# vandenheuvel/relp

Hardware: AMD Instinct MI355X
Metric: simplex pivots/sec + wall-clock to optimal, Netlib 25fv47 @1 GPU (higher is better)
Workload: dtype f64; 1 GPU; Netlib 25FV47 821x1876, steepest-edge pricing, explicit-inverse carry, exact certificate inside the timed step, no presolve (+520 virtual artificials); carry=explicit, refactors=0, parallelism=1 LP per GPU x1, certified=True, objective_bits=1791

## Files before the change

relp_amd/csrc/kernels.hip:

```cpp
#include <hip/hip_runtime.h>
#include <hip/hip_ext.h>

#include <cmath>
#include <cstdlib>
#include <string>
#include <utility>

#include "kernels.hpp"
#include "pivot_step.hpp"
#include "price_step.hpp"
#include "solver.hpp"
#include "wave_ops.hpp"

namespace relp {


__global__ void budget_kernel(Ctl* ctl, long long add) {
    if (ctl->status == ST_BUDGET) ctl->status = ST_RUNNING;
    ctl->budget = ctl->iters + add;
}

typedef double f64x2_t __attribute__((ext_vector_type(2)));
template <int RULE, bool USE_LDS, int LPC, bool UNIT = false>
__global__ void __launch_bounds__(256) price_kernel(DeviceLP lp, int skip_weights, double tol_dual, int col_first,
// ... 1796 lines not shown
            ctl->rho_buf ^= 1;
        }
        s_toggle = toggle;
        s_amount = amount;
    }
    __syncthreads();
    const int toggle = s_toggle;
    if (toggle >= 0) {
        const double amount = s_amount;
        for (int e = lp.col_start[toggle] + threadIdx.x; e < lp.col_start[toggle + 1]; e += blockDim.x)
            lp.rhs[lp.row_index[e]] -= amount * lp.value[e];
    }
}

constexpr int K2F_NW = K2F_THREADS / WAVE;
constexpr int K2F_INLINE_BLOCKS = 128;

struct K2fShared {
    double akey[K2F_NW];
    unsigned long long arank[K2F_NW];
    double red[K2F_NW + 2];
    double red2[K2F_NW + 2];
    double cbarv[K2F_MAX_BLOCKS];
    int crows[K2F_INLINE_BLOCKS * ELL_W];
    double cvals[K2F_INLINE_BLOCKS * ELL_W];
    int clen[K2F_INLINE_BLOCKS];
    int rows[K2_COL_CHUNK];
    double vals[K2_COL_CHUNK];
    double bcast[4];
    int ibcast[2];
};
static_assert(K2F_INLINE_BLOCKS * ELL_W <= 2 * K2F_THREADS, "the inline entries are two loads per thread");
struct K2fCandidateLoads {
    int j, len;
    double key, cbar;
    int row[2];
    double val[2];
};
__device__ __forceinline__ void k2f_candidates_issue(const DeviceLP& lp, int n_price_blocks, K2fCandidateLoads& c) {
    const int tid = threadIdx.x;
    const int bc = tid < n_price_blocks ? tid : 0;
    c.j = lp.cand_j[bc];
    c.key = lp.cand_key[bc];
    c.cbar = lp.cand_cbar[bc];
    c.len = lp.cand_len[bc];
#pragma unroll
    for (int t = 0; t < 2; ++t) {
        const int e = tid + t * K2F_THREADS;
        const int ec = e < n_price_blocks * ELL_W ? e : 0;
        c.row[t] = lp.cand_rows[ec];
        c.val[t] = lp.cand_vals[ec];
    }
}
template <int RULE>
__device__ __forceinline__ void k2f_candidates_fold(const DeviceLP& lp, int n_price_blocks, K2fShared& sm, const K2fCandidateLoads& c,
                                                    double& ckey, unsigned long long& crank) {
    const int tid = threadIdx.x;
    if (tid < n_price_blocks) {
        sm.cbarv[tid] = c.cbar;
        offer_entering<RULE>(c.key, c.j, tid, ckey, crank);
    }
    if (n_price_blocks <= K2F_INLINE_BLOCKS) {
#pragma unroll
        for (int t = 0; t < 2; ++t) {
            const int e = tid + t * K2F_THREADS;
            if (e < n_price_blocks * ELL_W) {
                sm.crows[e] = c.row[t];
                sm.cvals[e] = c.val[t];
            }
        }
        if (tid < n_price_blocks) sm.clen[tid] = c.len;
    }
    for (int b = tid + K2F_THREADS; b < n_price_blocks; b += K2F_THREADS) {
        const int j = lp.cand_j[b];
        const double k = lp.cand_key[b];
        const double cb = lp.cand_cbar[b];
        RELP_LOADS_ISSUED();
        sm.cbarv[b] = cb;
        offer_entering<RULE>(k, j, b, ckey, crank);
    }
}
template <int RULE>
__device__ __forceinline__ int k2f_entering(double ckey, unsigned long long crank, K2fShared& sm, double& cbar_q, int& winner_block) {
    const int q = entering_winner<RULE>(ckey, crank, sm.akey, sm.arank, winner_block);
    cbar_q = q >= 0 ? sm.cbarv[winner_block] : 0.0;
    return q;
}
template <int R>
__device__ __forceinline__ void k2f_ftran_inline(const DeviceLP& lp, const double* T, const K2fShared& sm, int q, int winner_block,
                                                 double (&al)[R], int& ca, int& cb_) {
    const int tid = threadIdx.x, m = lp.m, ld = lp.ld;
    const int len = sm.clen[winner_block];
    if (len >= 0) {
        constexpr int G = R <= 4 ? R : 4;
#pragma unroll
        for (int rg = 0; rg < R; rg += G) {
            double t[G][ELL_W];
#pragma unroll
            for (int g = 0; g < G; ++g) {
                const int i = tid + (rg + g) * K2F_THREADS;
                const double* col = T + (i < m ? i : 0);
#pragma unroll
                for (int e = 0; e < ELL_W; ++e) t[g][e] = col[(size_t)sm.crows[winner_block * ELL_W + e] * ld];
            }
            RELP_LOADS_ISSUED();
#pragma unroll
            for (int g = 0; g < G; ++g) {
                double a0 = 0.0;
#pragma unroll
                for (int e = 0; e < ELL_W; ++e) a0 += t[g][e] * sm.cvals[winner_block * ELL_W + e];
                if (tid + (rg + g) * K2F_THREADS < m) al[rg + g] = a0;
            }
        }
    }
    if (len > ELL_W || len < 0) {
        ca = lp.col_start[q] + (len < 0 ? 0 : ELL_W);
        cb_ = lp.col_start[q + 1];
    }
}
template <int R>
__device__ __forceinline__ void k2f_ftran_csc(const DeviceLP& lp, const double* T, K2fShared& sm, int ca, int cb_, double (&al)[R]) {
    const int tid = threadIdx.x, m = lp.m, ld = lp.ld;
    for (int c0 = ca; c0 < cb_; c0 += K2_COL_CHUNK) {
        const int cnt = min(K2_COL_CHUNK, cb_ - c0);
        __syncthreads();
        for (int e = tid; e < cnt; e += K2F_THREADS) {
            sm.rows[e] = lp.row_index[c0 + e];
            sm.vals[e] = lp.value[c0 + e];
        }
        __syncthreads();
        if constexpr (R <= 8) {
            double acc[R][4];
            int row[R];
#pragma unroll
            for (int r = 0; r < R; ++r) {
                const int i = tid + r * K2F_THREADS;
                row[r] = i < m ? i : 0;
                acc[r][0] = acc[r][1] = acc[r][2] = acc[r][3] = 0.0;
            }
            int e = 0;
            for (; e + 4 <= cnt; e += 4) {
                const size_t o0 = (size_t)sm.rows[e] * ld, o1 = (size_t)sm.rows[e + 1] * ld, o2 = (size_t)sm.rows[e + 2] * ld, o3 = (size_t)sm.rows[e + 3] * ld;
                const double v0 = sm.vals[e], v1 = sm.vals[e + 1], v2 = sm.vals[e + 2], v3 = sm.vals[e + 3];
                double x[R][4];
#pragma unroll
                for (int r = 0; r < R; ++r) {
                    x[r][0] = T[o0 + row[r]];
                    x[r][1] = T[o1 + row[r]];
                    x[r][2] = T[o2 + row[r]];
                    x[r][3] = T[o3 + row[r]];
                }
#pragma unroll
                for (int r = 0; r < R; ++r) {
                    acc[r][0] += x[r][0] * v0;
                    acc[r][1] += x[r][1] * v1;
                    acc[r][2] += x[r][2] * v2;
                    acc[r][3] += x[r][3] * v3;
                }
            }
            for (; e < cnt; ++e) {
                const size_t o = (size_t)sm.rows[e] * ld;
                const double v = sm.vals[e];
                double x[R];
#pragma unroll
                for (int r = 0; r < R; ++r) x[r] = T[o + row[r]];
#pragma unroll
                for (int r = 0; r < R; ++r) acc[r][0] += x[r] * v;
            }
#pragma unroll
            for (int r = 0; r < R; ++r)
                if (tid + r * K2F_THREADS < m) al[r] += (acc[r][0] + acc[r][1]) + (acc[r][2] + acc[r][3]);
        } else {
#pragma unroll
            for (int r = 0; r < R; ++r) {
                const int i = tid + r * K2F_THREADS;
                if (i >= m) continue;
                const double* col = T + i;
                double a0 = 0.0, a1 = 0.0, a2 = 0.0, a3 = 0.0;
                int e = 0;
                for (; e + 4 <= cnt; e += 4) {
                    a0 += col[(size_t)sm.rows[e] * ld] * sm.vals[e];
                    a1 += col[(size_t)sm.rows[e + 1] * ld] * sm.vals[e + 1];
                    a2 += col[(size_t)sm.rows[e + 2] * ld] * sm.vals[e + 2];
                    a3 += col[(size_t)sm.rows[e + 3] * ld] * sm.vals[e + 3];
                }
                for (; e < cnt; ++e) a0 += col[(size_t)sm.rows[e] * ld] * sm.vals[e];
                al[r] += (a0 + a1) + (a2 + a3);
            }
        }
    }
}
template <int R>
__device__ __forceinline__ void k2f_pass1(const DeviceLP& lp, bool bounded, const double (&al)[R], const double (&xb)[R], const int (&bas)[R],
                                          double tol_pivot, double slack, int skip_artificial_rows, bool (&eligible)[R], double (&room)[R],
                                          double& sumsq, double& theta) {
    const int tid = threadIdx.x, m = lp.m;
#pragma unroll
    for (int r = 0; r < R; ++r) {
        const int i = tid + r * K2F_THREADS;
        const double a = al[r];
        sumsq += a * a;
        const bool allowed = i < m && !(skip_artificial_rows && bas[r] < lp.n_art);
        const RowRoom row = row_room(a, xb[r], [&] { return lp.xub[i]; }, allowed, bounded, tol_pivot);
        eligible[r] = row.eligible;
        room[r] = row.room;
        if (row.eligible) theta = fmin(theta, harris_pass1(row.room, slack, a));
    }
}
__device__ __forceinline__ void k2f_reduce(K2fShared& sm, double sumsq, double theta, double& gamma_q, double& theta_max) {
    const int lane = threadIdx.x & (WAVE - 1), wave = threadIdx.x / WAVE;
    sumsq = wave_sum(sumsq);
    theta = wave_min(theta);
    if (lane == LAST) {
        sm.red[wave] = sumsq;
        sm.red2[wave] = theta;
    }
    __syncthreads();
    if (wave == 0) {
        double t1 = lane < K2F_NW ? sm.red[lane] : 0.0;
        double t2 = lane < K2F_NW ? sm.red2[lane] : INFINITY;
        t1 = wave_sum(t1);
        t2 = wave_min(t2);
        if (lane == LAST) {
            sm.red[K2F_NW] = t1;
            sm.red2[K2F_NW] = t2;
        }
    }
    __syncthreads();
    gamma_q = 1.0 + sm.red[K2F_NW];
    theta_max = sm.red2[K2F_NW];
}
template <int R>
__device__ __forceinline__ int k2f_pass2(bool textbook, const double (&al)[R], const bool (&eligible)[R], const double (&room)[R],
                                         const int (&bas)[R], double theta_max, K2fShared& sm) {
    double hkey = 0.0;
    unsigned long long hrank = RANK_NONE;
#pragma unroll
    for (int r = 0; r < R; ++r) {
        const double mag = fabs(al[r]);
        if (eligible[r] && harris_accepts(room[r], mag, theta_max))
            keep_better(harris_key(textbook, mag), leaving_rank(bas[r], threadIdx.x + r * K2F_THREADS), hkey, hrank);
    }
    block_argbest(hkey, hrank, sm.akey, sm.arank);
    return leaving_row(hrank);
}
template <int R>
__device__ __forceinline__ void k2f_broadcast_row(int p, const double (&al)[R], const double (&xb)[R], const double (&room)[R],
                                                  const int (&bas)[R], K2fShared& sm) {
#pragma unroll
    for (int r = 0; r < R; ++r) {
        if ((int)threadIdx.x + r * K2F_THREADS == p) {
            sm.bcast[1] = al[r];
            sm.bcast[2] = xb[r];
            sm.bcast[3] = room[r];
            sm.ibcast[0] = bas[r];
        }
    }
    __syncthreads();
}

template <int RULE, int R>
__global__ void __launch_bounds__(K2F_THREADS) ftran_ratio_fast_kernel(DeviceLP lp, int n_price_blocks, double tol_pivot,
                                                                     double harris_delta, int skip_artificial_rows,
                                                                     int mode, int n_alpha_slices) {
    __shared__ K2fShared sm;
    Ctl* ctl = lp.ctl;
    STAMP_INIT;
    const int tid = threadIdx.x;
    const int m = lp.m;
    kernel_args_ready(ctl, lp.xB, lp.basis, lp.alpha_in, lp.cand_j, lp.cand_key, lp.cand_cbar, lp.cand_len, lp.cand_rows, lp.cand_vals, m, n_price_blocks,
                      n_alpha_slices);
    double xb[R];
    int bas[R];
    double ain[R];
    const bool preselected = n_alpha_slices > 0;
    const double* ain_from = preselected ? lp.alpha_in : lp.xB;
#pragma unroll
    for (int r = 0; r < R; ++r) {
        const int i = tid + r * K2F_THREADS;
        const int ic = i < m ? i : 0;
        xb[r] = lp.xB[ic];
        bas[r] = lp.basis[ic];
        ain[r] = ain_from[ic];
    }
    double ckey = 0.0;
    unsigned long long crank = RANK_NONE;
    K2fCandidateLoads cand;
    k2f_candidates_issue(lp, n_price_blocks, cand);
    RELP_LOADS_PINNED();
    const int status = ctl->status;
    const long long iters = ctl->iters;
    const long long budget = ctl->budget;
    const int forced_q = ctl->forced_q;
    const int forced_p = ctl->forced_p;
    const double minus_obj = ctl->minus_obj;
    const int q_loaded = ctl->q;
    const double cbar_loaded = ctl->cbar_q;
    RELP_LOADS_ISSUED();
    const int q_pre = preselected ? q_loaded : -1;
    const double cbar_pre = preselected ? cbar_loaded : 0.0;
#pragma unroll
    for (int r = 0; r < R; ++r) {
        if (tid + r * K2F_THREADS >= m) {
            xb[r] = 0.0;
            bas[r] = 0x7fffffff;
        }
        if (!preselected || tid + r * K2F_THREADS >= m) ain[r] = 0.0;
    }
    if (!preselected) k2f_candidates_fold<RULE>(lp, n_price_blocks, sm, cand, ckey, crank);
    const bool inline_column = forced_q < 0 && !preselected && n_price_blocks <= K2F_INLINE_BLOCKS;
    if (status != ST_RUNNING) return;
    STAMP(0);
    if (mode == 0 && iters >= budget) {
        if (tid == 0) ctl_budget(*ctl);
        return;
    }
    int q;
    double cbar_q;
    int winner_block = 0;
    if (preselected && forced_q < 0) {
        q = q_pre;
        cbar_q = cbar_pre;
    } else if (forced_q < 0) {
        q = k2f_entering<RULE>(ckey, crank, sm, cbar_q, winner_block);
    } else {
        q = forced_q;
// ... 102 lines not shown
        }
        __syncthreads();
        if (wave_k2 == 0) {
            int carry = 0;
#pragma unroll
            for (int base = 0; base < R * NW; base += WAVE) {
                const int c = base + lane_k2 < R * NW ? s_nz_count[base + lane_k2] : 0;
                int incl = c;
#pragma unroll
                for (int d = 1; d < WAVE; d <<= 1) {
                    const int up = __shfl_up(incl, d);
                    if (lane_k2 >= d) incl += up;
                }
                if (base + lane_k2 < R * NW) s_nz_count[base + lane_k2] = carry + incl - c;
                carry += __shfl(incl, WAVE - 1);
            }
            if (lane_k2 == 0) s_nz_count[R * NW] = carry;
        }
        __syncthreads();
#pragma unroll
        for (int r = 0; r < R; ++r) {
            const int i = tid + r * K2F_THREADS;
            if (i < m && (al[r] != 0.0 || i == p)) {
                const int slot = s_nz_count[r * NW + wave_k2] + __popcll(masks[r] & ((1ull << lane_k2) - 1ull));
                lp.nz_index[slot] = i;
                lp.nz_alpha[slot] = al[r];
            }
        }
        total = s_nz_count[R * NW];
    }
#pragma unroll
    for (int r = 0; r < R; ++r) {
        const int i = tid + r * K2F_THREADS;
        if (i < m) {
            lp.alpha[i] = al[r];
            lp.xB[i] = (i == p) ? xp : xb[r] - al[r] * xp;
        }
    }
    STAMP(5);
    const int leaving_flipped = bounded ? lp.flipped[leaving] : 0;
    if (step.leaves_at_upper) {
        const double sgn_l = leaving_flipped ? -1.0 : 1.0;
        for (int e = lp.col_start[leaving] + tid; e < lp.col_start[leaving + 1]; e += K2F_THREADS)
            lp.rhs[lp.row_index[e]] -= step.ub_leaving * sgn_l * lp.value[e];
    }
    if (bounded) __syncthreads();
    if (tid == 0) {
        lp.basis[p] = q;
        push_touched(lp, *ctl, p);
        if (lp.eta_cap > 0) {
            int is_new = 0;
            if (eta_slot_p < 0) {
                const int k = ctl->eta_count;
                lp.eta_slot[p] = k;
                lp.eta_rows[k] = p;
                ctl->eta_count = k + 1;
                is_new = 1;
            }
            ctl->eta_new = is_new;
            ctl->eta_version = ctl->eta_version + 1;
        }
        ctl_basis_change(lp, *ctl, bounded, q, p, leaving, leaving_flipped, step, ub_q, cbar_q, alpha_pq, gamma_q, total, minus_obj, iters);
        ctl->rho_buf ^= 1;
    }
    STAMP(6);
}

constexpr int KF_THREADS = K2F_THREADS;
constexpr int KF_NW = KF_THREADS / WAVE;
template <int RULE, int KF_R>
__global__ void __launch_bounds__(KF_THREADS) pivot_fused_kernel(DeviceLP lp, DeviceLP::State in, DeviceLP::State out, int n_price_blocks,
                                                                 double tol_pivot, double harris_delta, int skip_artificial_rows) {
    constexpr int R = KF_R;
    constexpr int KF_U = KF_R * KF_THREADS / WAVE;
    constexpr int KF_M = KF_R * KF_THREADS;
    __shared__ K2fShared sm;
    __shared__ double s_alpha[KF_M];
    const Ctl* ctl = in.ctl;
    const int tid = threadIdx.x;
    const int lane = tid & (WAVE - 1), wave = tid / WAVE;
#ifdef RELP_STAMPS
    unsigned long long t_prev__ = clock64();
    if (tid == 0 && blockIdx.x == 0) lp.dbg[63] += 1;
#define FSTAMP(k) do { if (tid == 0 && blockIdx.x == 0) { unsigned long long t__ = clock64(); lp.dbg[(k)] += t__ - t_prev__; t_prev__ = t__; } } while (0)
#else
#define FSTAMP(k) do {} while (0)
#endif
    const int m = lp.m, ld = lp.ld;
    const bool writer = blockIdx.x == 0;
    kernel_args_ready(ctl, in.xB, in.basis, lp.cand_j, lp.cand_key, lp.cand_cbar, lp.cand_len, lp.cand_rows, lp.cand_vals, m, n_price_blocks);
    double xb[R];
    int bas[R];
#pragma unroll
    for (int r = 0; r < R; ++r) {
        const int i = tid + r * KF_THREADS;
        const int ic = i < m ? i : 0;
        xb[r] = in.xB[ic];
        bas[r] = in.basis[ic];
    }
    double ckey = 0.0;
    unsigned long long crank = RANK_NONE;
    K2fCandidateLoads cand;
    k2f_candidates_issue(lp, n_price_blocks, cand);
    RELP_LOADS_PINNED();
    const int status = ctl->status;
    const long long iters = ctl->iters;
    const long long budget = ctl->budget;
    const double minus_obj = ctl->minus_obj;
    const int t_buf = ctl->t_buf;
    RELP_LOADS_ISSUED();
#pragma unroll
    for (int r = 0; r < R; ++r) {
        if (tid + r * KF_THREADS >= m) {
            xb[r] = 0.0;
            bas[r] = 0x7fffffff;
        }
    }
    k2f_candidates_fold<RULE>(lp, n_price_blocks, sm, cand, ckey, crank);
    const bool inline_column = n_price_blocks <= K2F_INLINE_BLOCKS;
    auto hand_on = [&](auto verdict) {
        if (!writer) return;
#pragma unroll
        for (int r = 0; r < R; ++r) {
            const int i = tid + r * KF_THREADS;
            if (i < m) {
                out.xB[i] = xb[r];
                out.basis[i] = bas[r];
            }
        }
        if (tid == 0) {
            Ctl c;
            ctl_copy(c, *ctl);
            verdict(c);
            c.forced_q = -1;
            c.forced_p = -1;
            ctl_copy(*out.ctl, c);
        }
    };
    if (status != ST_RUNNING) {
        hand_on([](Ctl&) {});
        return;
    }
    FSTAMP(0);
    if (iters >= budget) {
        hand_on([](Ctl& c) { ctl_budget(c); });
        return;
    }
    const int j_own = blockIdx.x * KF_NW + wave;
    const bool own = j_own < m;
    const double* t_old = (t_buf ? lp.Binv2 : lp.Binv);
    double* t_new = (t_buf ? lp.Binv : lp.Binv2);
    const double* c_old = t_old + (size_t)(own ? j_own : 0) * ld;
    double o[KF_U];
#pragma unroll
    for (int u = 0; u < KF_U; ++u) {
        const int i = lane + u * WAVE;
        o[u] = c_old[i < m ? i : 0];
    }
    double pi_old = lp.minus_pi[own ? j_own : 0];
    RELP_LOADS_PINNED();
    double cbar_q;
    int winner_block = 0;
    const int q = k2f_entering<RULE>(ckey, crank, sm, cbar_q, winner_block);
    if (q < 0) {
        hand_on([](Ctl& c) { ctl_no_entering(c, 0); });
        return;
    }
    FSTAMP(1);
    double al[R];
#pragma unroll
    for (int r = 0; r < R; ++r) al[r] = 0.0;
    int ca = 0, cb_ = 0;
    if (inline_column) {
        k2f_ftran_inline<R>(lp, t_old, sm, q, winner_block, al, ca, cb_);
    } else {
        ca = lp.col_start[q];
        cb_ = lp.col_start[q + 1];
    }
#pragma unroll
    for (int u = 0; u < KF_U; ++u) {
        if (!own || lane + u * WAVE >= m) o[u] = 0.0;
    }
    if (!own || lane != LAST) pi_old = 0.0;
    k2f_ftran_csc<R>(lp, t_old, sm, ca, cb_, al);
    FSTAMP(2);
    const HarrisRule harris = harris_rule(harris_delta);
    double sumsq = 0.0, theta = INFINITY;
    bool eligible[R];
    double room[R];
    k2f_pass1<R>(lp, false, al, xb, bas, tol_pivot, harris.slack, skip_artificial_rows, eligible, room, sumsq, theta);
#pragma unroll
    for (int r = 0; r < R; ++r) s_alpha[tid + r * KF_THREADS] = al[r];
    double gamma_q, theta_max;
    k2f_reduce(sm, sumsq, theta, gamma_q, theta_max);
    FSTAMP(3);
    const int p = k2f_pass2<R>(harris.textbook, al, eligible, room, bas, theta_max, sm);
    if (p < 0) {
        hand_on([q](Ctl& c) { ctl_unbounded(c, q, 0); });
        return;
    }
    FSTAMP(4);
    k2f_broadcast_row<R>(p, al, xb, room, bas, sm);
    const double alpha_pq = sm.bcast[1];
    const int leaving = sm.ibcast[0];
    const Step step = step_decision(false, false, p, alpha_pq, sm.bcast[2], sm.bcast[3], INFINITY);
    const double xp = step.xp;
    if (writer) {
#pragma unroll
        for (int r = 0; r < R; ++r) {
            const int i = tid + r * KF_THREADS;
            if (i < m) {
                lp.alpha[i] = al[r];
                out.xB[i] = (i == p) ? xp : xb[r] - al[r] * xp;
                out.basis[i] = (i == p) ? q : bas[r];
            }
        }
        if (tid == 0) {
            Ctl c;
            ctl_copy(c, *ctl);
            ctl_basis_change(lp, c, false, q, p, leaving, 0, step, INFINITY, cbar_q, alpha_pq, gamma_q, 0, minus_obj, iters);
            c.t_buf = t_buf ^ 1;
            ctl_copy(*out.ctl, c);
        }
    }
    FSTAMP(5);
    if (!own) return;
    const int u_p = p >> 6, lane_p = p & (WAVE - 1);
    double o_p = 0.0;
#pragma unroll
    for (int u = 0; u < KF_U; ++u) o_p = (u == u_p) ? o[u] : o_p;
    const double r_j = __shfl(o_p, lane_p) / alpha_pq;
    double* c_new = t_new + (size_t)j_own * ld;
    double w_j = 0.0;
    double a_u[KF_U];
#pragma unroll
    for (int u = 0; u < KF_U; ++u) a_u[u] = s_alpha[lane + u * WAVE];
    __builtin_amdgcn_sched_barrier(0);
#pragma unroll
    for (int u = 0; u < KF_U; ++u) {
        const int i = lane + u * WAVE;
        const double a = a_u[u];
        w_j += a * o[u];
        if (i < m) c_new[i] = (i == p) ? r_j : ((a != 0.0) ? o[u] - a * r_j : o[u]);
    }
    w_j = wave_sum(w_j);
    if (lane == LAST) {
        lp.w[j_own] = w_j;
        lp.rho[j_own] = r_j;
        lp.minus_pi[j_own] = pi_old - cbar_q * r_j;
    }
    FSTAMP(6);
}
#undef FSTAMP
__global__ void __launch_bounds__(256) begin_batch_kernel(DeviceLP lp, long long add) {
    const DeviceLP::State s0 = lp.state[0];
    for (int i = threadIdx.x; i < lp.m; i += 256) {
        s0.xB[i] = lp.xB[i];
        s0.basis[i] = lp.basis[i];
    }
    if (threadIdx.x == 0) {
        Ctl c = *lp.ctl;
        if (c.status == ST_BUDGET) c.status = ST_RUNNING;
        c.budget = c.iters + add;
        *lp.ctl = c;
        *s0.ctl = c;
    }
}
__global__ void __launch_bounds__(256) commit_kernel(DeviceLP lp, int parity) {
    const DeviceLP::State last = lp.state[parity];
    const int t_buf = last.ctl->t_buf;
    const int m = lp.m, ld = lp.ld;
    if (t_buf) {
        const int lane = threadIdx.x & (WAVE - 1);
        for (int j = blockIdx.x * 4 + threadIdx.x / WAVE; j < m; j += gridDim.x * 4) {
            const double* src = lp.Binv2 + (size_t)j * ld;
            double* dst = lp.Binv + (size_t)j * ld;
            for (int i = lane; i < m; i += WAVE) dst[i] = src[i];
        }
    }
    if (blockIdx.x == 0) {
        for (int i = threadIdx.x; i < m; i += 256) {
            lp.xB[i] = last.xB[i];
            lp.basis[i] = last.basis[i];
        }
        if (threadIdx.x == 0) {
            Ctl c = *last.ctl;
            c.t_buf = 0;
            *lp.ctl = c;
            if (lp.ctl_mirror) {
                *lp.ctl_mirror = c;
                __threadfence_system();
            }
        }
    }
}

constexpr int K3_THREADS = 256;
constexpr int K3_CPW = 2;
constexpr int K3_SMALL_NZ = 32;
template <bool EAGER>
__global__ void __launch_bounds__(K3_THREADS) update_kernel(DeviceLP lp) {
    Ctl* ctl = lp.ctl;
    const int m = lp.m, ld = lp.ld;
    const int lane = threadIdx.x & (WAVE - 1);
    const int wave = threadIdx.x / WAVE;
    int slot0 = (blockIdx.x * (K3_THREADS / WAVE) + wave) * K3_CPW;
    int j0 = slot0, j1 = slot0 + 1;
    bool two = slot0 + 1 < m;
    int row_lo = 0, row_hi = m;
    bool split = false;
    if (!EAGER && lp.track_touched) {
        if (ctl->status != ST_RUNNING || !ctl->pending) return;
        for (int j = blockIdx.x * K3_THREADS + threadIdx.x; j < m; j += gridDim.x * K3_THREADS)
            if (!lp.touched[j]) {
                const double a_j = lp.alpha[j];
                lp.w[j] = a_j;
                lp.rho[j] = 0.0;
                if (lp.prw) {
                    lp.prw[(size_t)4 * j + 1] = 0.0;
                    lp.prw[(size_t)4 * j + 2] = a_j;
                }
                if (lp.rho_nz) lp.rho_nz[j] = 0;
            }
        const int n_touched = ctl->touched_count;
        const int nz_small = ctl->nz_count;
        if (nz_small > 0 && nz_small <= K3_SMALL_NZ) {
            const int slot = (blockIdx.x * (K3_THREADS / WAVE) + wave) * 8 + (lane >> 3);
            if ((slot & ~7) >= n_touched) return;
            const bool active = slot < n_touched;
            const int sub = lane & 7;
            const int j = lp.tlist[active ? slot : 0];
            double* c = lp.Binv + (size_t)j * ld;
            const int p = ctl->p;
            const double alpha_pq = ctl->alpha_pq;
// ... 575 lines not shown
    }
}

void launch_price_dense(const DeviceLP& d, const KernelPath& path, int skip_weights, double tol, hipStream_t s) {
    const size_t lds = (size_t)3 * d.dense_ld * sizeof(double);
    const dim3 grid(path.dense_blocks), lane_block(dense_lane_threads(d.m)), row_block(K1D_THREADS);
    const int cand_offset = path.price_blocks;
    switch (path.dense_storage) {
    case DenseStorage::NONE: throw std::logic_error("launch_price_dense: no dense block");
    case DenseStorage::F64_LANE: RELP_LAUNCH(0, price_dense_lane_kernel<8>, grid, lane_block, 0, s, d, skip_weights, tol, cand_offset); break;
    case DenseStorage::F32_LANE: RELP_LAUNCH(0, price_dense_lane_kernel<4>, grid, lane_block, 0, s, d, skip_weights, tol, cand_offset); break;
    case DenseStorage::I8_LANE: RELP_LAUNCH(0, price_dense_lane_kernel<1>, grid, lane_block, 0, s, d, skip_weights, tol, cand_offset); break;
    case DenseStorage::I8_PERMUTED: RELP_LAUNCH(0, (price_dense_kernel<false, true>), grid, row_block, lds, s, d, skip_weights, tol, cand_offset); break;
    case DenseStorage::F32_ROWS: RELP_LAUNCH(0, price_dense_kernel<true>, grid, row_block, lds, s, d, skip_weights, tol, cand_offset); break;
    case DenseStorage::F64_ROWS: RELP_LAUNCH(0, price_dense_kernel<false>, grid, row_block, lds, s, d, skip_weights, tol, cand_offset); break;
    }
}
static void allow_full_lds(const void* kernel) {
    hipFuncAttributes attr{};
    size_t fixed = 0;
    if (hipFuncGetAttributes(&attr, kernel) == hipSuccess) fixed = attr.sharedSizeBytes;
    if (hipFuncSetAttribute(kernel, hipFuncAttributeMaxDynamicSharedMemorySize, (int)(160 * 1024 - fixed)) != hipSuccess) (void)hipGetLastError();
}
void configure_dense_lds() {
    static PerDeviceOnce once;
    once.run([] {
        allow_full_lds(reinterpret_cast<const void*>(&price_dense_kernel<false>));
        allow_full_lds(reinterpret_cast<const void*>(&price_dense_kernel<true>));
        allow_full_lds(reinterpret_cast<const void*>(&price_dense_kernel<false, true>));
    });
}
void launch_ftran_partial(const DeviceLP& d, int n_slices, int n_price_blocks, int rule, hipStream_t s) {
    hipLaunchKernelGGL(ftran_partial_kernel, dim3((d.m + 255) / 256, n_slices), dim3(256), 0, s, d, n_slices, n_price_blocks, rule);
}

void configure_lds() {
    static PerDeviceOnce once;
    once.run([] {
        allow_full_lds(reinterpret_cast<const void*>(&price_kernel<RELP_PIVOT_STEEPEST_EDGE, true, PRICE_LPC>));
        allow_full_lds(reinterpret_cast<const void*>(&price_kernel<RELP_PIVOT_DANTZIG, true, PRICE_LPC>));
        allow_full_lds(reinterpret_cast<const void*>(&price_kernel<RELP_PIVOT_FIRST_PROFITABLE, true, PRICE_LPC>));
        allow_full_lds(reinterpret_cast<const void*>(&price_kernel<RELP_PIVOT_FIRST_PROFITABLE_MEMORY, true, PRICE_LPC>));
    });
}

template <int RULE>
static void launch_ftran_ratio_rule(const DeviceLP& d, const KernelPath& path, double tol_pivot, double harris_delta, int skip_artificial_rows,
                                    int mode, int n_alpha_slices, hipStream_t s) {
    const RatioKernel kernel = mode == 0 ? path.ratio_kernel : path.ratio_kernel_no_change;
    const int n_price_blocks = path.slots();
    if (n_alpha_slices > 0 && ratio_rows_per_thread(kernel) == 0) throw std::logic_error("launch_ftran_ratio: a preselected alpha needs the register-resident ratio test");
#define RELP_RATIO_REGISTERS(R) \
    RELP_LAUNCH(1, (ftran_ratio_fast_kernel<RULE, R>), dim3(1), dim3(K2F_THREADS), 0, s, d, n_price_blocks, tol_pivot, harris_delta, skip_artificial_rows, mode, n_alpha_slices)
    switch (kernel) {
    case RatioKernel::REGISTERS_2: RELP_RATIO_REGISTERS(2); break;
    case RatioKernel::REGISTERS_4: RELP_RATIO_REGISTERS(4); break;
    case RatioKernel::REGISTERS_8: RELP_RATIO_REGISTERS(8); break;
    case RatioKernel::REGISTERS_16: RELP_RATIO_REGISTERS(16); break;
    case RatioKernel::MULTI_WORKGROUP: {
        const int blocks = (d.m + K2L_THREADS - 1) / K2L_THREADS;
        RELP_LAUNCH(1, (k2l_ftran_kernel<RULE>), dim3(blocks), dim3(K2L_THREADS), 0, s, d, n_price_blocks, tol_pivot, harris_delta, skip_artificial_rows);
        hipLaunchKernelGGL(k2l_harris_kernel, dim3(blocks), dim3(K2L_THREADS), 0, s, d, blocks, tol_pivot, skip_artificial_rows);
        hipLaunchKernelGGL(k2l_apply_kernel, dim3(blocks), dim3(K2L_THREADS), 0, s, d, blocks);
        break;
    }
    case RatioKernel::ONE_WORKGROUP:
        RELP_LAUNCH(1, (ftran_ratio_kernel<RULE>), dim3(1), dim3(K2_THREADS), 0, s, d, n_price_blocks, tol_pivot, harris_delta, skip_artificial_rows, mode);
        break;
    }
#undef RELP_RATIO_REGISTERS
}

void launch_ftran_ratio(const DeviceLP& d, const KernelPath& path, int rule, double tol_pivot, double harris_delta, int skip_artificial_rows,
                        int mode, int n_alpha_slices, hipStream_t s) {
    if (rule == RELP_PIVOT_STEEPEST_EDGE)
        launch_ftran_ratio_rule<RELP_PIVOT_STEEPEST_EDGE>(d, path, tol_pivot, harris_delta, skip_artificial_rows, mode, n_alpha_slices, s);
    else
        launch_ftran_ratio_rule<RELP_PIVOT_DANTZIG>(d, path, tol_pivot, harris_delta, skip_artificial_rows, mode, n_alpha_slices, s);
}

template <int RULE>
static void launch_pivot_fused_rule(const DeviceLP& d, const KernelPath& path, int parity, double tol_pivot, double harris_delta,
                                    int skip_artificial_rows, hipStream_t s) {
    const dim3 grid((d.m + KF_NW - 1) / KF_NW);
    const int n_price_blocks = path.price_blocks;
    switch (path.fused_rows) {
    case 2: RELP_LAUNCH(1, (pivot_fused_kernel<RULE, 2>), grid, dim3(KF_THREADS), 0, s, d, d.state[parity], d.state[parity ^ 1], n_price_blocks, tol_pivot, harris_delta, skip_artificial_rows); break;
    case 4: RELP_LAUNCH(1, (pivot_fused_kernel<RULE, 4>), grid, dim3(KF_THREADS), 0, s, d, d.state[parity], d.state[parity ^ 1], n_price_blocks, tol_pivot, harris_delta, skip_artificial_rows); break;
    default: throw std::logic_error("launch_pivot_fused: the path has no fused pivot");
    }
}
void launch_pivot_fused(const DeviceLP& d, const KernelPath& path, int rule, int parity, double tol_pivot, double harris_delta,
                        int skip_artificial_rows, hipStream_t s) {
    if (rule == RELP_PIVOT_STEEPEST_EDGE) launch_pivot_fused_rule<RELP_PIVOT_STEEPEST_EDGE>(d, path, parity, tol_pivot, harris_delta, skip_artificial_rows, s);
    else launch_pivot_fused_rule<RELP_PIVOT_DANTZIG>(d, path, parity, tol_pivot, harris_delta, skip_artificial_rows, s);
}
void launch_begin_batch(const DeviceLP& d, long long add, hipStream_t s) {
    hipLaunchKernelGGL(begin_batch_kernel, dim3(1), dim3(256), 0, s, d, add);
}
void launch_commit(const DeviceLP& d, int parity, hipStream_t s) {
    hipLaunchKernelGGL(commit_kernel, dim3(std::min(256, (d.m + 3) / 4)), dim3(256), 0, s, d, parity);
}

void launch_update(const DeviceLP& d, const KernelPath& path, hipStream_t s) {
    const int cols_per_block = (K3_THREADS / WAVE) * K3_CPW;
    const dim3 grid((d.m + cols_per_block - 1) / cols_per_block), grid_split((d.m + K3_CPW - 1) / K3_CPW);
    switch (path.update_kernel) {
    case UpdateKernel::EAGER: RELP_LAUNCH(2, (update_kernel<true>), grid, dim3(K3_THREADS), 0, s, d); break;
    case UpdateKernel::PREDICATED: RELP_LAUNCH(2, (update_kernel<false>), grid, dim3(K3_THREADS), 0, s, d); break;
    case UpdateKernel::PREDICATED_SPLIT_GRID: RELP_LAUNCH(2, (update_kernel<false>), grid_split, dim3(K3_THREADS), 0, s, d); break;
    }
}

void launch_budget(const DeviceLP& d, long long add, hipStream_t s) {
    hipLaunchKernelGGL(budget_kernel, dim3(1), dim3(1), 0, s, d.ctl, add);
}

void launch_pi(const DeviceLP& d, hipStream_t s) {
    hipLaunchKernelGGL(cb_kernel, dim3(1), dim3(CB_THREADS), 0, s, d);
    hipLaunchKernelGGL(pi_kernel, dim3((d.m + 3) / 4), dim3(256), 0, s, d);
    hipLaunchKernelGGL(pi_sparse_kernel, dim3((d.m + 255) / 256), dim3(256), 0, s, d);
}
void launch_cb(const DeviceLP& d, hipStream_t s) { hipLaunchKernelGGL(cb_kernel, dim3(1), dim3(CB_THREADS), 0, s, d); }
void launch_k2l_preselected(const DeviceLP& d, double tol_pivot, double harris_delta, int skip_artificial_rows, hipStream_t s) {
    const int blocks = (d.m + K2L_THREADS - 1) / K2L_THREADS;
    hipLaunchKernelGGL(k2l_preselected_kernel, dim3(blocks), dim3(K2L_THREADS), 0, s, d, tol_pivot, harris_delta, skip_artificial_rows);
    hipLaunchKernelGGL(k2l_harris_kernel, dim3(blocks), dim3(K2L_THREADS), 0, s, d, blocks, tol_pivot, skip_artificial_rows);
    hipLaunchKernelGGL(k2l_apply_kernel, dim3(blocks), dim3(K2L_THREADS), 0, s, d, blocks);
}
void launch_xb(const DeviceLP& d, hipStream_t s) {
    hipLaunchKernelGGL(xb_kernel, dim3((d.m + WAVE - 1) / WAVE), dim3(256), 0, s, d);
}
void launch_gamma_init(const DeviceLP& d, int identity, hipStream_t s) {
    hipLaunchKernelGGL(gamma_init_kernel, dim3(d.n - d.n_art), dim3(256), 0, s, d, identity);
}
void launch_identity(double* X, int m, int ld, hipStream_t s) {
    hipLaunchKernelGGL(identity_kernel, dim3((m + 255) / 256, std::min(m, 65535)), dim3(256), 0, s, X, m, ld);
}
__global__ void __launch_bounds__(256) scatter_kernel(double* X, const long long* index, const double* value, long long count) {
    const long long stride = (long long)gridDim.x * 256;
    for (long long e = (long long)blockIdx.x * 256 + threadIdx.x; e < count; e += stride) X[index[e]] = value[e];
}
void launch_scatter(double* X, const long long* index, const double* value, long long count, hipStream_t s) {
    if (count <= 0) return;
    hipLaunchKernelGGL(scatter_kernel, dim3((unsigned)std::min<long long>(4096, (count + 255) / 256)), dim3(256), 0, s, X, index, value, count);
}
void launch_residual(const DeviceLP& d, const double* T, double* S, hipStream_t s) {
    hipLaunchKernelGGL(residual_kernel, dim3(d.m), dim3(256), 0, s, d, T, S);
}
__global__ void __launch_bounds__(256) copy_rows_kernel(const double* src, double* dst, int m, int ld, const int* row_list, int n_rows) {
    const int i = blockIdx.x * 256 + threadIdx.x;
    if (i >= m) return;
    for (int idx = blockIdx.y; idx < n_rows; idx += gridDim.y) {
        const size_t row = (size_t)row_list[idx] * ld;
        dst[row + i] = src[row + i];
    }
}
void launch_copy_rows(const double* src, double* dst, int m, int ld, const int* row_list, int n_rows, hipStream_t s) {
    if (n_rows > 0) hipLaunchKernelGGL(copy_rows_kernel, dim3((m + 255) / 256, std::min(n_rows, 65535)), dim3(256), 0, s, src, dst, m, ld, row_list, n_rows);
}
void launch_gemm_polish(PolishGemm gemm, const double* X, const double* R, double* C, int m, int ld, const int* row_list, int n_rows, hipStream_t s) {
    const int rows = row_list ? n_rows : m;
    if (rows <= 0) return;
    dim3 grid((m + GT - 1) / GT, (rows + GT - 1) / GT);
    if (gemm == PolishGemm::MFMA) hipLaunchKernelGGL((gemm_mfma_kernel<0>), grid, dim3(256), 0, s, X, R, C, m, ld, (double*)nullptr, row_list, n_rows);
    else hipLaunchKernelGGL((gemm_polish_kernel<0>), grid, dim3(256), 0, s, X, R, C, m, ld, (double*)nullptr);
}
// ... 48 lines not shown
```

relp_amd/csrc/price_step.hpp:

```cpp
#pragma once
#include "pivot_step.hpp"

namespace relp {

__device__ __forceinline__ bool column_priced(int pos, bool bounded = true) { return pos == -1 || (bounded && pos == -2); }
__device__ __forceinline__ double column_sign(int pos, bool bounded = true) { return (bounded && pos == -2) ? -1.0 : 1.0; }

__device__ __forceinline__ double weight_after_pivot(double gam, double d_rho, double d_w, double gamma_q, double alpha_pq, bool is_leaving) {
    if (is_leaving) return gamma_q / (alpha_pq * alpha_pq);
    const double sq = d_rho * d_rho;
    gam = gam - 2.0 * d_rho * d_w + sq * gamma_q;
    gam = fmax(gam, 1.0 + sq);
    return gam;
}

template <int RULE>
__device__ __forceinline__ double price_key(double cbar, double tol_dual, double gam, int j, int last, int n, bool& candidate) {
    candidate = cbar < -tol_dual;
    if (RULE == RELP_PIVOT_STEEPEST_EDGE) return cbar * cbar / gam;
    if (RULE == RELP_PIVOT_DANTZIG) return -cbar;
    if (RULE == RELP_PIVOT_FIRST_PROFITABLE) return -(double)j;
    if (last >= 0 && j == last) candidate = false;
    const long long rank = (last < 0) ? j : (j > last ? (long long)j - last - 1 : (long long)j + n - last);
    return -(double)rank;
}

template <int RULE>
__device__ __forceinline__ unsigned long long entering_rank(int j, int block) {
    const unsigned long long order = (RULE == RELP_PIVOT_STEEPEST_EDGE) ? (unsigned long long)(0x7fffffff - j) : (unsigned long long)j;
    return (order << 16) | (unsigned long long)block;
}
template <int RULE>
__device__ __forceinline__ int entering_column(unsigned long long rank) {
    const int order = (int)(rank >> 16);
    return (RULE == RELP_PIVOT_STEEPEST_EDGE) ? 0x7fffffff - order : order;
}
__device__ __forceinline__ int entering_block(unsigned long long rank) { return (int)(rank & 0xffff); }
template <int RULE>
__device__ __forceinline__ void offer_entering(double key, int j, int block, double& best_key, unsigned long long& best_rank) {
    if (j >= 0) keep_better(key, entering_rank<RULE>(j, block), best_key, best_rank);
}
__device__ __forceinline__ Cand no_candidate(int aux = 0) {
    Cand c;
    c.key = 0.0;
    c.idx = -1;
    c.aux = aux;
    return c;
}
template <int RULE>
__device__ __forceinline__ bool offer_candidate(Cand& best, double key, int j) {
    Cand c;
    c.key = key;
    c.idx = j;
    c.aux = 0;
    best = (RULE == RELP_PIVOT_STEEPEST_EDGE) ? better<TIE_LARGER_IDX>(best, c) : better<TIE_SMALLER_IDX>(best, c);
    return best.idx == j;
}
template <int RULE>
__device__ __forceinline__ Cand block_best_candidate(Cand best, Cand* s) {
    return (RULE == RELP_PIVOT_STEEPEST_EDGE) ? block_best<TIE_LARGER_IDX>(best, s) : block_best<TIE_SMALLER_IDX>(best, s);
}

__device__ __forceinline__ void publish_candidate(const DeviceLP& lp, int slot, double key, int j, double cbar, int len) {
    lp.cand_key[slot] = key;
    lp.cand_j[slot] = j;
    lp.cand_cbar[slot] = cbar;
    lp.cand_len[slot] = len;
}
__device__ __forceinline__ void publish_entry(const DeviceLP& lp, int slot, int e, int row, double val) {
    lp.cand_rows[(size_t)slot * ELL_W + e] = row;
    lp.cand_vals[(size_t)slot * ELL_W + e] = val;
}
__device__ __forceinline__ void publish_no_candidate(const DeviceLP& lp, int slot) { lp.cand_j[slot] = -1; }

template <int RULE>
__device__ __forceinline__ void fold_candidates(const int* cand_j, const double* cand_key, int n_blocks, int tid, int n_threads,
                                                double& key, unsigned long long& rank) {
    for (int b = tid; b < n_blocks; b += n_threads) offer_entering<RULE>(cand_key[b], cand_j[b], b, key, rank);
}
template <int RULE>
__device__ __forceinline__ int entering_winner(double key, unsigned long long rank, double* s_key, unsigned long long* s_rank, int& block) {
    block_argbest(key, rank, s_key, s_rank);
    if (rank == RANK_NONE) return -1;
    block = entering_block(rank);
    return entering_column<RULE>(rank);
}

__device__ __forceinline__ double reduced_cost_of(double cost_q, const int* col_start, const int* row_index, const double* value,
                                                  const double* minus_pi, int q) {
    double cb = cost_q;
    for (int e = col_start[q]; e < col_start[q + 1]; ++e) cb += value[e] * minus_pi[row_index[e]];
    return cb;
}

}
```

relp_amd/csrc/wave_ops.hpp:

```cpp
#pragma once
#include <hip/hip_runtime.h>
#include <cmath>
#include "solver.hpp"

namespace relp {

#ifdef RELP_STAMPS
#define STAMP(k) do { if (threadIdx.x == 0) { unsigned long long t__ = clock64(); lp.dbg[(k)] += t__ - t_prev__; t_prev__ = t__; } } while (0)
#define STAMP_INIT unsigned long long t_prev__ = clock64(); if (threadIdx.x == 0) lp.dbg[63] += 1
#else
#define STAMP(k) do {} while (0)
#define STAMP_INIT do {} while (0)
#endif

template <class A>
__device__ __forceinline__ void kernel_arg_ready(A a) { asm volatile("" ::"s"(a)); }
template <class... A>
__device__ __forceinline__ void kernel_args_ready(A... a) { (kernel_arg_ready(a), ...); }
#define RELP_LOADS_PINNED() asm volatile("" ::: "memory")
#define RELP_LOADS_ISSUED() do { asm volatile("" ::: "memory"); __builtin_amdgcn_sched_barrier(0); } while (0)

struct Cand {
    double key;
    int idx;
// ... 3 lines not shown
enum : int { TIE_LARGER_IDX = 0, TIE_SMALLER_IDX = 1, TIE_SMALLER_AUX = 2 };

template <int TIE>
__device__ __forceinline__ Cand better(Cand a, Cand b) {
    bool take_b;
    if (TIE == TIE_LARGER_IDX) take_b = (b.key > a.key) | ((b.key == a.key) & (b.idx > a.idx));
    else if (TIE == TIE_SMALLER_IDX) take_b = (b.key > a.key) | ((b.key == a.key) & (b.idx < a.idx));
    else take_b = (b.key > a.key) | ((b.key == a.key) & ((b.aux < a.aux) | ((b.aux == a.aux) & (b.idx < a.idx))));
    take_b = (a.idx < 0) | ((b.idx >= 0) & take_b);
    Cand r;
    r.key = take_b ? b.key : a.key;
    r.idx = take_b ? b.idx : a.idx;
    r.aux = take_b ? b.aux : a.aux;
    return r;
}

constexpr int DPP_QUAD_1032 = 0xB1;
constexpr int DPP_QUAD_2301 = 0x4E;
constexpr int DPP_ROW_HALF_MIRROR = 0x141;
constexpr int DPP_ROW_ROR4 = 0x124;
constexpr int DPP_ROW_ROR8 = 0x128;
constexpr int DPP_ROW_BCAST15 = 0x142;
constexpr int DPP_ROW_BCAST31 = 0x143;

template <int CTRL, int ROW_MASK>
__device__ __forceinline__ int dpp_i32(int old, int v) {
    return __builtin_amdgcn_update_dpp(old, v, CTRL, ROW_MASK, 0xF, false);
}
template <int CTRL, int ROW_MASK>
__device__ __forceinline__ double dpp_f64(double old, double v) {
    const int lo = dpp_i32<CTRL, ROW_MASK>(__double2loint(old), __double2loint(v));
    const int hi = dpp_i32<CTRL, ROW_MASK>(__double2hiint(old), __double2hiint(v));
    return __hiloint2double(hi, lo);
}
template <int CTRL, int ROW_MASK>
__device__ __forceinline__ Cand dpp_cand(Cand v) {
    Cand o;
    o.key = dpp_f64<CTRL, ROW_MASK>(v.key, v.key);
    o.idx = dpp_i32<CTRL, ROW_MASK>(v.idx, v.idx);
    o.aux = dpp_i32<CTRL, ROW_MASK>(v.aux, v.aux);
    return o;
}

template <int CTRL, int ROW_MASK> __device__ __forceinline__ double dpp_move(double old, double v) { return dpp_f64<CTRL, ROW_MASK>(old, v); }
template <int CTRL, int ROW_MASK> __device__ __forceinline__ int dpp_move(int old, int v) { return dpp_i32<CTRL, ROW_MASK>(old, v); }
template <int CTRL, int ROW_MASK> __device__ __forceinline__ Cand dpp_move(Cand, Cand v) { return dpp_cand<CTRL, ROW_MASK>(v); }
template <int CTRL, int ROW_MASK> __device__ __forceinline__ unsigned long long dpp_move(unsigned long long old, unsigned long long v) {
    const int lo = dpp_i32<CTRL, ROW_MASK>((int)(unsigned)old, (int)(unsigned)v);
    const int hi = dpp_i32<CTRL, ROW_MASK>((int)(unsigned)(old >> 32), (int)(unsigned)(v >> 32));
    return ((unsigned long long)(unsigned)hi << 32) | (unsigned)lo;
}
template <bool FILL_SELF, class T, class Op>
__device__ __forceinline__ T wave_ladder(T v, T neutral, Op op) {
    v = op(v, dpp_move<DPP_QUAD_1032, 0xF>(FILL_SELF ? v : neutral, v));
    v = op(v, dpp_move<DPP_QUAD_2301, 0xF>(FILL_SELF ? v : neutral, v));
    v = op(v, dpp_move<DPP_ROW_ROR4, 0xF>(FILL_SELF ? v : neutral, v));
    v = op(v, dpp_move<DPP_ROW_ROR8, 0xF>(FILL_SELF ? v : neutral, v));
    v = op(v, dpp_move<DPP_ROW_BCAST15, 0xA>(FILL_SELF ? v : neutral, v));
    v = op(v, dpp_move<DPP_ROW_BCAST31, 0xC>(FILL_SELF ? v : neutral, v));
    return v;
}
template <int TIE>
__device__ __forceinline__ Cand wave_best(Cand v) { return wave_ladder<true>(v, v, [](Cand a, Cand b) { return better<TIE>(a, b); }); }
__device__ __forceinline__ double wave_sum(double v) { return wave_ladder<false>(v, 0.0, [](double a, double b) { return a + b; }); }
__device__ __forceinline__ double wave_min(double v) { return wave_ladder<true>(v, v, [](double a, double b) { return fmin(a, b); }); }
constexpr int LAST = WAVE - 1;

__device__ __forceinline__ double wave_max(double v) { return wave_ladder<true>(v, v, [](double a, double b) { return fmax(a, b); }); }
__device__ __forceinline__ unsigned long long wave_min_u64(unsigned long long v) {
    return wave_ladder<true>(v, v, [](unsigned long long a, unsigned long long b) { return a < b ? a : b; });
}
__device__ __forceinline__ int wave_min_i32(int v) { return wave_ladder<true>(v, v, [](int a, int b) { return min(a, b); }); }
__device__ __forceinline__ double lane63_f64(double v) {
    const int lo = __builtin_amdgcn_readlane(__double2loint(v), 63);
    const int hi = __builtin_amdgcn_readlane(__double2hiint(v), 63);
    return __hiloint2double(hi, lo);
}
__device__ __forceinline__ unsigned long long lane63_u64(unsigned long long v) {
    const unsigned lo = (unsigned)__builtin_amdgcn_readlane((int)(unsigned)v, 63);
    const unsigned hi = (unsigned)__builtin_amdgcn_readlane((int)(unsigned)(v >> 32), 63);
    return ((unsigned long long)hi << 32) | lo;
}
constexpr unsigned long long RANK_NONE = ~0ull;
__device__ __forceinline__ void block_argbest(double& key, unsigned long long& rank, double* s_key, unsigned long long* s_rank) {
    const int lane = threadIdx.x & (WAVE - 1), wave = threadIdx.x / WAVE;
    const int nwaves = (blockDim.x + WAVE - 1) / WAVE;
    const double k0 = rank == RANK_NONE ? -INFINITY : key;
    const double wmax = lane63_f64(wave_max(k0));
    const unsigned long long tie = (rank != RANK_NONE && k0 == wmax) ? rank : RANK_NONE;
    const unsigned long long wmin = lane63_u64(wave_min_u64(tie));
    __syncthreads();
    if (lane == 0) {
        s_key[wave] = wmax;
        s_rank[wave] = wmin;
    }
    __syncthreads();
    double bk = -INFINITY;
    unsigned long long br = RANK_NONE;
    for (int wv = 0; wv < nwaves; ++wv) {
        const double k = s_key[wv];
        const unsigned long long r = s_rank[wv];
        const bool take = r != RANK_NONE && (br == RANK_NONE || k > bk || (k == bk && r < br));
        bk = take ? k : bk;
        br = take ? r : br;
    }
    key = bk;
    rank = br;
}

template <int TIE>
__device__ __forceinline__ Cand block_best(Cand v, Cand* s) {
    const int lane = threadIdx.x & (WAVE - 1);
    const int wave = threadIdx.x / WAVE;
    const int nwaves = (blockDim.x + WAVE - 1) / WAVE;
    v = wave_best<TIE>(v);
    __syncthreads();
    if (lane == LAST) {
        s[wave].key = v.key;
        s[wave].idx = v.idx;
        s[wave].aux = v.aux;
    }
    __syncthreads();
    if (wave == 0) {
        Cand t;
        t.key = 0.0;
        t.idx = -1;
        t.aux = 0;
        if (lane < nwaves) {
            t.key = s[lane].key;
            t.idx = s[lane].idx;
            t.aux = s[lane].aux;
        }
        t = wave_best<TIE>(t);
        if (lane == LAST) {
            s[nwaves].key = t.key;
            s[nwaves].idx = t.idx;
            s[nwaves].aux = t.aux;
        }
    }
    __syncthreads();
    Cand r;
    r.key = s[nwaves].key;
    r.idx = s[nwaves].idx;
    r.aux = s[nwaves].aux;
    return r;
}

template <int OP>
__device__ __forceinline__ double block_reduce(double v, double* s) {
    const int lane = threadIdx.x & (WAVE - 1);
    const int wave = threadIdx.x / WAVE;
    const int nwaves = (blockDim.x + WAVE - 1) / WAVE;
    v = OP == 0 ? wave_sum(v) : wave_min(v);
    __syncthreads();
    if (lane == LAST) s[wave] = v;
    __syncthreads();
    if (wave == 0) {
        double t = OP == 0 ? 0.0 : INFINITY;
        if (lane < nwaves) t = s[lane];
        t = OP == 0 ? wave_sum(t) : wave_min(t);
        if (lane == LAST) s[nwaves] = t;
    }
    __syncthreads();
    return s[nwaves];
}

}
```

Before: 58700 pivots/s.

## Dedicate block zero as pivot writer and trim barriers in fused pivot kernel

```diff
diff --git a/relp_amd/csrc/kernels.hip b/relp_amd/csrc/kernels.hip
--- a/relp_amd/csrc/kernels.hip
+++ b/relp_amd/csrc/kernels.hip
@@ -1902,7 +1902,7 @@
 }
 template <int RULE>
 __device__ __forceinline__ int k2f_entering(double ckey, unsigned long long crank, K2fShared& sm, double& cbar_q, int& winner_block) {
-    const int q = entering_winner<RULE>(ckey, crank, sm.akey, sm.arank, winner_block);
+    const int q = entering_winner<RULE, true>(ckey, crank, sm.akey, sm.arank, winner_block);
     cbar_q = q >= 0 ? sm.cbarv[winner_block] : 0.0;
     return q;
 }
@@ -2027,6 +2027,7 @@
         if (row.eligible) theta = fmin(theta, harris_pass1(row.room, slack, a));
     }
 }
+static_assert(K2F_NW == 8, "k2f_reduce spells out the ladder's tree over eight wave partials");
 __device__ __forceinline__ void k2f_reduce(K2fShared& sm, double sumsq, double theta, double& gamma_q, double& theta_max) {
     const int lane = threadIdx.x & (WAVE - 1), wave = threadIdx.x / WAVE;
     sumsq = wave_sum(sumsq);
@@ -2036,19 +2037,11 @@
         sm.red2[wave] = theta;
     }
     __syncthreads();
-    if (wave == 0) {
-        double t1 = lane < K2F_NW ? sm.red[lane] : 0.0;
-        double t2 = lane < K2F_NW ? sm.red2[lane] : INFINITY;
-        t1 = wave_sum(t1);
-        t2 = wave_min(t2);
-        if (lane == LAST) {
-            sm.red[K2F_NW] = t1;
-            sm.red2[K2F_NW] = t2;
-        }
-    }
-    __syncthreads();
-    gamma_q = 1.0 + sm.red[K2F_NW];
-    theta_max = sm.red2[K2F_NW];
+    const double a = (sm.red[0] + sm.red[1]) + (sm.red[2] + sm.red[3]);
+    const double b = (sm.red[4] + sm.red[5]) + (sm.red[6] + sm.red[7]);
+    gamma_q = 1.0 + (a + b);
+    theta_max = fmin(fmin(fmin(sm.red2[0], sm.red2[1]), fmin(sm.red2[2], sm.red2[3])),
+                     fmin(fmin(sm.red2[4], sm.red2[5]), fmin(sm.red2[6], sm.red2[7])));
 }
 template <int R>
 __device__ __forceinline__ int k2f_pass2(bool textbook, const double (&al)[R], const bool (&eligible)[R], const double (&room)[R],
@@ -2061,7 +2054,7 @@
         if (eligible[r] && harris_accepts(room[r], mag, theta_max))
             keep_better(harris_key(textbook, mag), leaving_rank(bas[r], threadIdx.x + r * K2F_THREADS), hkey, hrank);
     }
-    block_argbest(hkey, hrank, sm.akey, sm.arank);
+    block_argbest<true>(hkey, hrank, sm.akey, sm.arank);
     return leaving_row(hrank);
 }
 template <int R>
@@ -2330,7 +2323,7 @@
 #ifdef RELP_STAMPS
     unsigned long long t_prev__ = clock64();
     if (tid == 0 && blockIdx.x == 0) lp.dbg[63] += 1;
-#define FSTAMP(k) do { if (tid == 0 && blockIdx.x == 0) { unsigned long long t__ = clock64(); lp.dbg[(k)] += t__ - t_prev__; t_prev__ = t__; } } while (0)
+#define FSTAMP(k) do { if (tid == 0 && blockIdx.x <= 1) { unsigned long long t__ = clock64(); lp.dbg[(k) + 16 * blockIdx.x] += t__ - t_prev__; t_prev__ = t__; } } while (0)
 #else
 #define FSTAMP(k) do {} while (0)
 #endif
@@ -2394,8 +2387,8 @@
         hand_on([](Ctl& c) { ctl_budget(c); });
         return;
     }
-    const int j_own = blockIdx.x * KF_NW + wave;
-    const bool own = j_own < m;
+    const int j_own = ((int)blockIdx.x - 1) * KF_NW + wave;
+    const bool own = !writer && j_own < m;
     const double* t_old = (t_buf ? lp.Binv2 : lp.Binv);
     double* t_new = (t_buf ? lp.Binv : lp.Binv2);
     const double* c_old = t_old + (size_t)(own ? j_own : 0) * ld;
@@ -2448,12 +2441,13 @@
         return;
     }
     FSTAMP(4);
-    k2f_broadcast_row<R>(p, al, xb, room, bas, sm);
-    const double alpha_pq = sm.bcast[1];
-    const int leaving = sm.ibcast[0];
-    const Step step = step_decision(false, false, p, alpha_pq, sm.bcast[2], sm.bcast[3], INFINITY);
-    const double xp = step.xp;
     if (writer) {
+        k2f_broadcast_row<R>(p, al, xb, room, bas, sm);
+        const double alpha_pq = sm.bcast[1];
+        const int leaving = sm.ibcast[0];
+        const Step step = step_decision(false, false, p, alpha_pq, sm.bcast[2], sm.bcast[3], INFINITY);
+        const double xp = step.xp;
+        FSTAMP(5);
 #pragma unroll
         for (int r = 0; r < R; ++r) {
             const int i = tid + r * KF_THREADS;
@@ -2470,9 +2464,13 @@
             c.t_buf = t_buf ^ 1;
             ctl_copy(*out.ctl, c);
         }
-    }
-    FSTAMP(5);
+        FSTAMP(6);
+        return;
+    }
     if (!own) return;
+    const double alpha_pq = s_alpha[p];
+    int lane_again = lane;
+    asm volatile("" : "+v"(lane_again));
     const int u_p = p >> 6, lane_p = p & (WAVE - 1);
     double o_p = 0.0;
 #pragma unroll
@@ -2482,11 +2480,11 @@
     double w_j = 0.0;
     double a_u[KF_U];
 #pragma unroll
-    for (int u = 0; u < KF_U; ++u) a_u[u] = s_alpha[lane + u * WAVE];
+    for (int u = 0; u < KF_U; ++u) a_u[u] = s_alpha[lane_again + u * WAVE];
     __builtin_amdgcn_sched_barrier(0);
 #pragma unroll
     for (int u = 0; u < KF_U; ++u) {
-        const int i = lane + u * WAVE;
+        const int i = lane_again + u * WAVE;
         const double a = a_u[u];
         w_j += a * o[u];
         if (i < m) c_new[i] = (i == p) ? r_j : ((a != 0.0) ? o[u] - a * r_j : o[u]);
@@ -2497,7 +2495,7 @@
         lp.rho[j_own] = r_j;
         lp.minus_pi[j_own] = pi_old - cbar_q * r_j;
     }
-    FSTAMP(6);
+    FSTAMP(7);
 }
 #undef FSTAMP
 __global__ void __launch_bounds__(256) begin_batch_kernel(DeviceLP lp, long long add) {
@@ -3239,7 +3237,7 @@
 template <int RULE>
 static void launch_pivot_fused_rule(const DeviceLP& d, const KernelPath& path, int parity, double tol_pivot, double harris_delta,
                                     int skip_artificial_rows, hipStream_t s) {
-    const dim3 grid((d.m + KF_NW - 1) / KF_NW);
+    const dim3 grid((d.m + KF_NW - 1) / KF_NW + 1);
     const int n_price_blocks = path.price_blocks;
     switch (path.fused_rows) {
     case 2: RELP_LAUNCH(1, (pivot_fused_kernel<RULE, 2>), grid, dim3(KF_THREADS), 0, s, d, d.state[parity], d.state[parity ^ 1], n_price_blocks, tol_pivot, harris_delta, skip_artificial_rows); break;
diff --git a/relp_amd/csrc/price_step.hpp b/relp_amd/csrc/price_step.hpp
--- a/relp_amd/csrc/price_step.hpp
+++ b/relp_amd/csrc/price_step.hpp
@@ -78,9 +78,9 @@
                                                 double& key, unsigned long long& rank) {
     for (int b = tid; b < n_blocks; b += n_threads) offer_entering<RULE>(cand_key[b], cand_j[b], b, key, rank);
 }
-template <int RULE>
+template <int RULE, bool SLOTS_FREE = false>
 __device__ __forceinline__ int entering_winner(double key, unsigned long long rank, double* s_key, unsigned long long* s_rank, int& block) {
-    block_argbest(key, rank, s_key, s_rank);
+    block_argbest<SLOTS_FREE>(key, rank, s_key, s_rank);
     if (rank == RANK_NONE) return -1;
     block = entering_block(rank);
     return entering_column<RULE>(rank);
diff --git a/relp_amd/csrc/wave_ops.hpp b/relp_amd/csrc/wave_ops.hpp
--- a/relp_amd/csrc/wave_ops.hpp
+++ b/relp_amd/csrc/wave_ops.hpp
@@ -109,6 +109,7 @@
     return ((unsigned long long)hi << 32) | lo;
 }
 constexpr unsigned long long RANK_NONE = ~0ull;
+template <bool SLOTS_FREE = false>
 __device__ __forceinline__ void block_argbest(double& key, unsigned long long& rank, double* s_key, unsigned long long* s_rank) {
     const int lane = threadIdx.x & (WAVE - 1), wave = threadIdx.x / WAVE;
     const int nwaves = (blockDim.x + WAVE - 1) / WAVE;
@@ -116,7 +117,7 @@
     const double wmax = lane63_f64(wave_max(k0));
     const unsigned long long tie = (rank != RANK_NONE && k0 == wmax) ? rank : RANK_NONE;
     const unsigned long long wmin = lane63_u64(wave_min_u64(tie));
-    __syncthreads();
+    if (!SLOTS_FREE) __syncthreads();
     if (lane == 0) {
         s_key[wave] = wmax;
         s_rank[wave] = wmin;
```

Measured after the change: 60000 pivots/s, median of 6. 2.2% higher.
